# TDLdefA-QUN/Noise-Resilience-in-Discrete-Time-Crystal-Realizations-on-Quantum-Computers

Hardware: AMD Instinct MI355X
Metric: Floquet-periods×instances/sec at L=20; RZZ-kernel HBM GB/s vs peak (higher is better)
Workload: dtype f64

## Files before the change

noise-resilience-in-discrete-time-crystal-realizations-on-quantum-computers_amd/csrc/dtc_wavefront.hip:

```cpp
#include <hip/hip_runtime.h>

#include "dtc_device.h"
#include "dtc_kernels.h"
#include "dtc_wf_frame.h"

#ifndef DTC_WF_SPLIT
#define DTC_WF_SPLIT 1
#endif
#ifndef DTC_WF_WAVE_XCH
#define DTC_WF_WAVE_XCH 0
#endif
#ifndef DTC_WF_WG4
#define DTC_WF_WG4 1
#endif

namespace dtc {

template <int LAY>
__device__ __forceinline__ void wf_diag(double2 (&v)[kRegs], const double2* slot, int t,
                                        double2 fac, double2 e) {
  static_assert(LAY >= 0 && LAY <= 2, "tile layout");
  const double2 c = cmul(fac, e);
  const double2* tr = slot + (LAY == 1   ? wf_l1_reg_index(ybase<1>(t))
                              : LAY == 2 ? ((t >> 6) & 3)
                                         : ((t & 7) << 4));
  constexpr int kStep = LAY == 1 ? 2 : (LAY == 2 ? 4 : 1);
#pragma unroll
  for (int g = 0; g < kRegs; g += 4) {
#pragma unroll
    for (int r = g; r < g + 4; ++r) v[r] = cmul(v[r], cmul(c, tr[r * kStep]));
    __builtin_amdgcn_sched_barrier(0);
  }
}

template <int KIND>
__device__ __forceinline__ void wf_kick_lane3(double2 (&v)[kRegs], double f) {
  const long long sm = (KIND == kKindRY && (__lane_id() & 8)) ? (long long)(1ull << 63) : 0ll;
#pragma unroll
  for (int r = 0; r < kRegs; ++r) {
    const double px = xor_lane<8>(v[r].x), py = xor_lane<8>(v[r].y);
    if (KIND == kKindRX) {
      v[r] = make_double2(fma(f, v[r].x, -py), fma(f, v[r].y, px));
    } else {
      v[r] = make_double2(fma(f, v[r].x, __longlong_as_double(__double_as_longlong(px) ^ sm)),
                          fma(f, v[r].y, __longlong_as_double(__double_as_longlong(py) ^ sm)));
    }
  }
}

__host__ __device__ constexpr int wf_slot_ofs(bool two_lay, int st) {
  return two_lay ? st * kWfTabB : (st >> 1) * kWfTab + (st & 1) * kWfTabB;
}
__host__ __device__ constexpr int wf_tab_lds(bool two_lay) { return wf_slot_ofs(two_lay, kWfSteps + 1); }
static_assert(kWfTabB == 64 && kWfL1Reg == 64 && kWfTabA == kWfFetchTabA && (kWfSteps & 1) == 0,
              "the register tables of dtc_wf_frame.h");

__host__ __device__ constexpr bool wf_wg4(int qm0) {
  return ((DTC_WF_WG4 >> (qm0 == 8)) & 1) &&
         sizeof(double) * kHalfSlots + sizeof(double2) * wf_tab_lds(kWfT2Lay1 && qm0 == 8) <=
             160 * 1024 / 4;
}

template <int KIND, int QM0, bool SPLIT>
__global__ __launch_bounds__(kThreads, SPLIT ? (wf_wg4(QM0) ? 4 : 3) : 2) void dtc_wf_pass(WfArgs A) {
  constexpr bool kWg4 = SPLIT && wf_wg4(QM0);
  constexpr bool kTwoLay = kWfT2Lay1 && QM0 == 8;
  __shared__ double2 s_tile[SPLIT ? 1 : kTile];
  __shared__ double s_half[SPLIT ? kHalfSlots : 1];
  __shared__ double2 s_tab[kWg4 || !SPLIT ? wf_tab_lds(kTwoLay) : (kWfSteps + 1) * kWfTab];
  static_assert(!kWg4 || sizeof(s_half) + sizeof(s_tab) <= 160 * 1024 / 4, "four workgroups per CU");
  static_assert(wf_tab_lds(kTwoLay) <= (kWfSteps + 1) * kWfTab, "the padded form holds the tables");

  const int t = threadIdx.x;
  const int og = A.octet_bits;
  const int64_t b = og ? (((int64_t)blockIdx.y << 3) | (blockIdx.x & 7)) : (int64_t)blockIdx.y;
  const int64_t tile = og ? (int64_t)(blockIdx.x >> 3) : (int64_t)blockIdx.x;
  if (b >= A.batch) return;
  const int inst = (int)((A.batch_start + b) / A.n_traj);
  const int n = A.n_steps;
  constexpr int kOddLay = kTwoLay ? 1 : 0;

  TileMap M;
  M.c = A.c;
  M.s = A.s;
  M.cmask = (1 << A.c) - 1;
  const int mid = A.s - A.c;
  M.tbase = ((tile & (((int64_t)1 << mid) - 1)) << A.c) | ((tile >> mid) << (A.s + kTileBits - A.c));

  const int var = A.out_bit >= 0 ? (int)((M.tbase >> A.out_bit) & 1) : 0;
  const double2* tg = A.tab + ((int64_t)inst * (kWfSteps + 1) * 2 + var) * kWfTab;
  double2 stage[kWfSteps + 1];
#pragma unroll
  for (int st = 0; st <= kWfSteps; ++st) {
    const int lay = (st & 1) ? kOddLay : 2;
    stage[st] = make_double2(1.0, 0.0);
    if (t < wf_reg_size(lay) && ((A.dmask >> st) & 1))
      stage[st] = tg[st * 2 * kWfTab + wf_reg_base(lay) + t];
  }

  const int64_t sbase = state_base(b, A.state_len, og);
  const int64_t vofs = octet_spread(M.at(ybase<2>(t)), og);
  double2 v[kRegs];
  {
    const double2* src = A.src + sbase + vofs;
#pragma unroll
    for (int r = 0; r < kRegs; ++r) {
      const d2v w =
          __builtin_nontemporal_load((const d2v*)(src + octet_spread(M.rel(r << 8), og)));
      v[r] = make_double2(w.x, w.y);
    }
  }
  const RecScalar R0(A.recs + b * kRecPerState);
  const RecScalar R1(A.recs + ((int64_t)A.batch + b) * kRecPerState);
  const long long fxd = R1.bits(8 * kRecTotal + kWfMaskXD);
  const int fzx = R1.i(kRecTotal, kWfMaskZX);
  const int last = 31 - __builtin_clz(A.dmask | 1);
  auto wf_fetch = [&](auto lay, int st) {
    constexpr int LAY = decltype(lay)::value;
    double2 e = make_double2(1.0, 0.0);
    if ((A.dmask >> st) & 1) {
      const int fx = (int)(fxd >> (kTileBits * st)) & (kTile - 1);
      e = tg[st * 2 * kWfTab + wf_thr_fetch(LAY, ybase<LAY>(t), fx)];
      if (st == last && wf_thr_neg(LAY, ybase<LAY>(t), fzx & (kTile - 1)))
        e = make_double2(-e.x, -e.y);
    }
    return e;
  };
  using L0 = std::integral_constant<int, 0>;
  using L1 = std::integral_constant<int, 1>;
  using L2 = std::integral_constant<int, 2>;
  using LOdd = std::integral_constant<int, kOddLay>;
  double2 cn = wf_fetch(L2{}, 0);
  if (t < kWfTabA) {
    const int fz = fzx & (kTile - 1);
#pragma unroll
    for (int st = 0; st <= kWfSteps; ++st) {
      const int lay = (st & 1) ? kOddLay : 2;
      if (t >= wf_reg_size(lay) || !((A.dmask >> st) & 1)) continue;
      const int fx = (int)(fxd >> (kTileBits * st)) & (kTile - 1);
      const int j = t ^ wf_reg_xmask(lay, fx);
      const bool neg = st == last && (__popc(j & wf_reg_zmask(lay, fz)) & 1);
      s_tab[wf_slot_ofs(kTwoLay, st) + j] =
          neg ? make_double2(-stage[st].x, -stage[st].y) : stage[st];
    }
  }
  __syncthreads();

  double2 gf = cmul(make_double2(R0.d(kRecTotal, 0), R0.d(kRecTotal, 1)),
                    make_double2(R1.d(kRecTotal, 0), R1.d(kRecTotal, 1)));
  auto diag = [&](auto lay, int st, auto nlay, int nx) {
    if ((A.dmask >> st) & 1) {
      wf_diag<decltype(lay)::value>(v, s_tab + wf_slot_ofs(kTwoLay, st), t, gf, cn);
      gf = make_double2(1.0, 0.0);
    }
    if (nx <= kWfSteps) cn = wf_fetch(nlay, nx);
  };
  auto kick = [&](auto nib, int st) {
    constexpr int N = decltype(nib)::value;
    if (!(A.mask[st] & (0xFu << (4 * N)))) return;
    const RecScalar R(A.recs + ((int64_t)(st >> 1) * A.batch + b) * kRecPerState);
    apply_nibble<N, KIND, N == 0 ? QM0 : 15, true>(v, R, (st & 1) * kTileBits);
  };
  constexpr bool kWaveXch = DTC_WF_WAVE_XCH != 0;

  auto kick3 = [&](int st) {
    if (!(A.mask[st] & 8u)) return;
    const RecScalar R(A.recs + ((int64_t)(st >> 1) * A.batch + b) * kRecPerState);
    wf_kick_lane3<KIND>(v, R.d((st & 1) * kTileBits + 3, 3));
  };

  int st = 0;
#pragma unroll 1
  do {
    diag(L2{}, st, LOdd{}, st + 1);
    if (st < n) {
      kick(L2{}, st);
      xch_tile<SPLIT, 2, 1>(v, s_tile, s_half, t);
      kick(L1{}, st);
      if constexpr (kTwoLay) {
        kick3(st);
      } else {
        xch_tile<SPLIT, 1, 0, kWaveXch>(v, s_tile, s_half, t);
        kick(L0{}, st);
      }
      diag(LOdd{}, st + 1, L2{}, st + 2);
      if (st + 1 < n) {
        if constexpr (kTwoLay) {
          kick3(st + 1);
          kick(L1{}, st + 1);
        } else {
          kick(L0{}, st + 1);
          xch_tile<SPLIT, 0, 1, kWaveXch>(v, s_tile, s_half, t);
          kick(L1{}, st + 1);
        }
        xch_tile<SPLIT, 1, 2>(v, s_tile, s_half, t);
        kick(L2{}, st + 1);
      }
    }
    st += 2;
  } while (st <= n);
  if (n & 1) xch_tile<SPLIT, kOddLay, 2>(v, s_tile, s_half, t);
  if (!A.dmask) {
    const int fz = fzx & (kTile - 1);
    const double sg = (__popc(t & fz) & 1) ? -1.0 : 1.0;
#pragma unroll
    for (int r = 0; r < kRegs; ++r) {
      const double s = (__popc(r & (fz >> 8)) & 1) ? -sg : sg;
      v[r] = cmul(v[r], make_double2(s * gf.x, s * gf.y));
    }
  }
  {
    const int fx = (fzx >> 16) & (kTile - 1);
    const int xr = fx >> 8;
    double2* dst = A.dst + sbase + octet_spread(M.at(ybase<2>(t) ^ (fx & 255)), og);
#pragma unroll
    for (int r = 0; r < kRegs; ++r) {
      d2v x;
      x.x = v[r].x;
      x.y = v[r].y;
      __builtin_nontemporal_store(x, (d2v*)(dst + octet_spread(M.rel((r ^ xr) << 8), og)));
    }
  }
}

hipError_t launch_wavefront(const WfArgs& a, int kind, hipStream_t stream) {
  if (a.L_eff < kTileBits || a.L_eff > 32 || a.n_steps < 1 || a.n_steps > kWfSteps ||
      a.c < 0 || a.c > kTileBits || a.s < a.c || a.s + kTileBits - a.c > a.L_eff ||
      a.out_bit >= a.L_eff || a.batch < 1 || !a.tab || !a.recs || !a.src || !a.dst)
    return hipErrorInvalidValue;
  if (a.octet_bits && (a.octet_bits < 4 || a.octet_bits > a.L_eff)) return hipErrorInvalidValue;
  const bool cols3 = a.c == 3;
  if (!cols3 && a.c != kTileBits) return hipErrorInvalidValue;
  for (int st = 0; st < a.n_steps; ++st)
    if (a.mask[st] >> kTileBits || (cols3 && (a.mask[st] & 7u))) return hipErrorInvalidValue;
  if (a.dmask < 0 || a.dmask >> (a.n_steps + 1)) return hipErrorInvalidValue;
  const int n_tiles = 1 << (a.L_eff - kTileBits);
  const dim3 grid = a.octet_bits ? dim3(n_tiles * 8, (a.batch + 7) / 8) : dim3(n_tiles, a.batch);
  const dim3 block(kThreads);
  constexpr bool kSplit = DTC_WF_SPLIT != 0;
  if (kind == kKindRX) {
    if (cols3) hipLaunchKernelGGL((dtc_wf_pass<kKindRX, 8, kSplit>), grid, block, 0, stream, a);
    else hipLaunchKernelGGL((dtc_wf_pass<kKindRX, 15, kSplit>), grid, block, 0, stream, a);
  } else if (kind == kKindRY) {
    if (cols3) hipLaunchKernelGGL((dtc_wf_pass<kKindRY, 8, kSplit>), grid, block, 0, stream, a);
    else hipLaunchKernelGGL((dtc_wf_pass<kKindRY, 15, kSplit>), grid, block, 0, stream, a);
  } else {
    return hipErrorInvalidValue;
  }
  return hipGetLastError();
}

}
```

noise-resilience-in-discrete-time-crystal-realizations-on-quantum-computers_amd/csrc/dtc_wf_frame.h:

```cpp
#pragma once
#include <stdint.h>

#ifdef __HIPCC__
#define DTC_WF_HD __host__ __device__
#else
#define DTC_WF_HD
#endif

namespace dtc {

static constexpr int kWfFrameSteps = 4;
static constexpr int kWfFrameBits = 12;

struct WfFrame {
  double coef[kWfFrameSteps][kWfFrameBits];
  uint64_t xdiag;
  int zlast;
  int xend;
  int ph;
};

DTC_WF_HD inline int wf_step_bits(uint32_t mask, int act) {
  int m = 0;
  for (int n = 0; n < 3; ++n)
    if (mask & (0xFu << (4 * n))) m |= 0xF << (4 * n);
  return m & act;
}

DTC_WF_HD inline void wf_frame_walk(bool rx, int n_steps, const uint32_t* mask, int dmask,
                                    int act, const int (*var)[kWfFrameBits],
                                    const double (*coef)[kWfFrameBits], WfFrame& o) {
  auto form_a = [&](int st, int k) { return (var[st][k] >> 1) ^ 1; };
  auto zbit = [&](int st, int k) {
    return rx ? (var[st][k] & 1) : ((var[st][k] & 1) ^ form_a(st, k));
  };
  int last = n_steps;
  for (int st = 0; st < n_steps; ++st)
    if ((dmask >> st) & 1) last = st;
  if ((dmask >> n_steps) & 1) last = n_steps;
  int npost = 0;
  for (int st = last; st < n_steps; ++st) {
    const int bits = wf_step_bits(mask[st], act);
    for (int k = 0; k < kWfFrameBits; ++k)
      if ((bits >> k) & 1) npost ^= zbit(st, k) << k;
  }
  int x = 0, z = 0, ph = 0;
  o.xdiag = 0;
  o.zlast = 0;
  for (int st = 0; st <= n_steps; ++st) {
    if ((dmask >> st) & 1) o.xdiag |= (uint64_t)x << (kWfFrameBits * st);
    if (st == last) {
      o.zlast = z ^ npost;
      z = npost;
    }
    for (int k = 0; k < kWfFrameBits; ++k) {
      if (st < kWfFrameSteps) o.coef[st][k] = 0.0;
      if (st == n_steps || !((wf_step_bits(mask[st], act) >> k) & 1)) continue;
      const int fa = form_a(st, k), n2 = zbit(st, k);
      const double g = fa ? -coef[st][k] : coef[st][k];
      const int flip = ((rx ? z : (x ^ z)) >> k) & 1;
      o.coef[st][k] = flip ? -g : g;
      ph += (rx ? 3 * fa : 2 * fa) + 2 * flip;
      x ^= fa << k;
      ph += 2 * (n2 & (x >> k) & 1);
      z ^= n2 << k;
    }
  }
  for (int st = n_steps + 1; st < kWfFrameSteps; ++st)
    for (int k = 0; k < kWfFrameBits; ++k) o.coef[st][k] = 0.0;
  o.xend = x;
  o.ph = ph & 3;
}

static constexpr int kWfL1Reg = 64;
static constexpr int kWfL1Thr = 32;

DTC_WF_HD inline bool wf_l1_reg_bit(int k) { return k >= 4 && k <= 7; }
DTC_WF_HD inline int wf_l1_reg_pos(int k) { return (k >= 3 && k <= 8) ? k - 3 : -1; }
DTC_WF_HD inline int wf_l1_thr_pos(int k) { return k == 3 ? 0 : ((k >= 8 && k <= 11) ? k - 7 : -1); }
DTC_WF_HD inline int wf_l1_reg_index(int y) { return (y >> 3) & 63; }
DTC_WF_HD inline int wf_l1_thr_index(int y) { return ((y >> 3) & 1) | (((y >> 8) & 15) << 1); }
DTC_WF_HD inline int wf_l1_reg_zmask(int z) { return (z >> 3) & 63; }
DTC_WF_HD inline int wf_l1_thr_zmask(int z) { return ((z >> 9) & 7) << 2; }
DTC_WF_HD inline bool wf_l1_in_reg(int k, int k2) {
  return wf_l1_reg_bit(k) || (k2 >= 0 && wf_l1_reg_bit(k2));
}

static constexpr int kWfFetchTabA = 128;
DTC_WF_HD inline int wf_thr_staged(int lay, int y) {
  return lay == 2 ? (y & (kWfFetchTabA - 1)) : (lay == 0 ? ((y >> 6) & 63) : wf_l1_thr_index(y));
}
DTC_WF_HD inline int wf_thr_fetch(int lay, int y, int fx) {
  const int i = wf_thr_staged(lay, y);
  if (lay == 2) return i ^ (fx & (kWfFetchTabA - 1));
  if (lay == 0) return kWfFetchTabA + (i ^ ((fx >> 6) & 63));
  return kWfL1Reg + (i ^ wf_l1_thr_index(fx));
}
DTC_WF_HD inline bool wf_thr_neg(int lay, int y, int fz) {
  const int zm = lay == 2 ? (fz & 63) : (lay == 0 ? ((fz >> 6) & 63) : wf_l1_thr_zmask(fz));
  int p = wf_thr_staged(lay, y) & zm;
  p ^= p >> 4;
  p ^= p >> 2;
  p ^= p >> 1;
  return p & 1;
}
DTC_WF_HD inline int wf_reg_base(int lay) { return lay == 2 ? kWfFetchTabA : 0; }
DTC_WF_HD inline int wf_reg_size(int lay) { return lay == 0 ? kWfFetchTabA : 64; }
DTC_WF_HD inline int wf_reg_xmask(int lay, int fx) {
  return lay == 2 ? ((fx >> 6) & 63) : (lay == 0 ? (fx & (kWfFetchTabA - 1)) : wf_l1_reg_index(fx));
}
DTC_WF_HD inline int wf_reg_zmask(int lay, int fz) {
  return lay == 2 ? ((fz >> 6) & 63) : (lay == 0 ? (fz & 63) : wf_l1_reg_zmask(fz));
}

}
#undef DTC_WF_HD
```

Measured before the change: 301,500.

## Add opt-in swap-based tile layout for split QM0=15 pass and pad layout-0 tables

Adds an optional layout path for the split kernel when QM0 is 15. It uses in-register lane swaps plus a single half-precision-slot LDS exchange, with pairwise kicks, in place of two tile exchanges per step. This aims to cut LDS traffic and barriers. Separately, the layout-0 diagonal tables in LDS are now padded (one slot per 16) to reduce bank conflicts, which changes the table stride and LDS footprint. The new exchange path is behind a compile flag that defaults off, and a host-visible symbol reports which form was built.

New measurement: 306,300, median of 6. +1.6%, better.

```diff
diff --git a/noise-resilience-in-discrete-time-crystal-realizations-on-quantum-computers_amd/csrc/dtc_wavefront.hip b/noise-resilience-in-discrete-time-crystal-realizations-on-quantum-computers_amd/csrc/dtc_wavefront.hip
--- a/noise-resilience-in-discrete-time-crystal-realizations-on-quantum-computers_amd/csrc/dtc_wavefront.hip
+++ b/noise-resilience-in-discrete-time-crystal-realizations-on-quantum-computers_amd/csrc/dtc_wavefront.hip
@@ -13,17 +13,21 @@
 #ifndef DTC_WF_WG4
 #define DTC_WF_WG4 1
 #endif
+#ifndef DTC_WF_T1_SWAP
+#define DTC_WF_T1_SWAP 0
+#endif
 
 namespace dtc {
 
-template <int LAY>
+template <int LAY, bool T1Q = false>
 __device__ __forceinline__ void wf_diag(double2 (&v)[kRegs], const double2* slot, int t,
                                         double2 fac, double2 e) {
-  static_assert(LAY >= 0 && LAY <= 2, "tile layout");
+  static_assert(LAY >= 0 && LAY <= 2 && (!T1Q || LAY == 0), "tile layout");
   const double2 c = cmul(fac, e);
   const double2* tr = slot + (LAY == 1   ? wf_l1_reg_index(ybase<1>(t))
                               : LAY == 2 ? ((t >> 6) & 3)
-                                         : ((t & 7) << 4));
+                              : T1Q      ? wf_pad0(wf_t1_ybase(kWfLayQ, t) & 0x70)
+                                         : wf_pad0((t & 7) << 4));
   constexpr int kStep = LAY == 1 ? 2 : (LAY == 2 ? 4 : 1);
 #pragma unroll
   for (int g = 0; g < kRegs; g += 4) {
@@ -48,8 +52,30 @@
   }
 }
 
+template <int FROM, int TO>
+__device__ __forceinline__ void exchange_t1(double2 (&v)[kRegs], double* s_half, int t) {
+  int bf = wf_t1_slot(wf_t1_ybase(FROM, t)), bt = wf_t1_slot(wf_t1_ybase(TO, t));
+  asm volatile("" : "+v"(bf), "+v"(bt));
+#pragma unroll
+  for (int r = 0; r < kRegs; ++r) s_half[bf ^ wf_t1_slot(wf_t1_roff(FROM, r))] = v[r].x;
+  __syncthreads();
+#pragma unroll
+  for (int r = 0; r < kRegs; ++r) v[r].x = s_half[bt ^ wf_t1_slot(wf_t1_roff(TO, r))];
+  __syncthreads();
+#pragma unroll
+  for (int r = 0; r < kRegs; ++r) s_half[bf ^ wf_t1_slot(wf_t1_roff(FROM, r))] = v[r].y;
+  __syncthreads();
+#pragma unroll
+  for (int r = 0; r < kRegs; ++r) v[r].y = s_half[bt ^ wf_t1_slot(wf_t1_roff(TO, r))];
+}
+
+__device__ __forceinline__ void wf_t1_swap(double2 (&v)[kRegs]) {
+  swap_reg_lane<0, 16>(v);
+  swap_reg_lane<1, 32>(v);
+}
+
 __host__ __device__ constexpr int wf_slot_ofs(bool two_lay, int st) {
-  return two_lay ? st * kWfTabB : (st >> 1) * kWfTab + (st & 1) * kWfTabB;
+  return two_lay ? st * kWfTabB : (st >> 1) * (kWfTabB + kWfTabA0) + (st & 1) * kWfTabB;
 }
 __host__ __device__ constexpr int wf_tab_lds(bool two_lay) { return wf_slot_ofs(two_lay, kWfSteps + 1); }
 static_assert(kWfTabB == 64 && kWfL1Reg == 64 && kWfTabA == kWfFetchTabA && (kWfSteps & 1) == 0,
@@ -65,6 +91,7 @@
 __global__ __launch_bounds__(kThreads, SPLIT ? (wf_wg4(QM0) ? 4 : 3) : 2) void dtc_wf_pass(WfArgs A) {
   constexpr bool kWg4 = SPLIT && wf_wg4(QM0);
   constexpr bool kTwoLay = kWfT2Lay1 && QM0 == 8;
+  constexpr bool kT1Swap = DTC_WF_T1_SWAP != 0 && SPLIT && QM0 == 15;
   __shared__ double2 s_tile[SPLIT ? 1 : kTile];
   __shared__ double s_half[SPLIT ? kHalfSlots : 1];
   __shared__ double2 s_tab[kWg4 || !SPLIT ? wf_tab_lds(kTwoLay) : (kWfSteps + 1) * kWfTab];
@@ -117,12 +144,12 @@
   const int last = 31 - __builtin_clz(A.dmask | 1);
   auto wf_fetch = [&](auto lay, int st) {
     constexpr int LAY = decltype(lay)::value;
+    const int yb = (kT1Swap && LAY == 0) ? wf_t1_ybase(kWfLayQ, t) : ybase<LAY>(t);
     double2 e = make_double2(1.0, 0.0);
     if ((A.dmask >> st) & 1) {
       const int fx = (int)(fxd >> (kTileBits * st)) & (kTile - 1);
-      e = tg[st * 2 * kWfTab + wf_thr_fetch(LAY, ybase<LAY>(t), fx)];
-      if (st == last && wf_thr_neg(LAY, ybase<LAY>(t), fzx & (kTile - 1)))
-        e = make_double2(-e.x, -e.y);
+      e = tg[st * 2 * kWfTab + wf_thr_fetch(LAY, yb, fx)];
+      if (st == last && wf_thr_neg(LAY, yb, fzx & (kTile - 1))) e = make_double2(-e.x, -e.y);
     }
     return e;
   };
@@ -140,7 +167,7 @@
       const int fx = (int)(fxd >> (kTileBits * st)) & (kTile - 1);
       const int j = t ^ wf_reg_xmask(lay, fx);
       const bool neg = st == last && (__popc(j & wf_reg_zmask(lay, fz)) & 1);
-      s_tab[wf_slot_ofs(kTwoLay, st) + j] =
+      s_tab[wf_slot_ofs(kTwoLay, st) + (lay == 0 ? wf_pad0(j) : j)] =
           neg ? make_double2(-stage[st].x, -stage[st].y) : stage[st];
     }
   }
@@ -150,7 +177,8 @@
                     make_double2(R1.d(kRecTotal, 0), R1.d(kRecTotal, 1)));
   auto diag = [&](auto lay, int st, auto nlay, int nx) {
     if ((A.dmask >> st) & 1) {
-      wf_diag<decltype(lay)::value>(v, s_tab + wf_slot_ofs(kTwoLay, st), t, gf, cn);
+      constexpr int LAY = decltype(lay)::value;
+      wf_diag<LAY, kT1Swap && LAY == 0>(v, s_tab + wf_slot_ofs(kTwoLay, st), t, gf, cn);
       gf = make_double2(1.0, 0.0);
     }
     if (nx <= kWfSteps) cn = wf_fetch(nlay, nx);
@@ -161,6 +189,14 @@
     const RecScalar R(A.recs + ((int64_t)(st >> 1) * A.batch + b) * kRecPerState);
     apply_nibble<N, KIND, N == 0 ? QM0 : 15, true>(v, R, (st & 1) * kTileBits);
   };
+  auto kick_pair = [&](auto half, int st) {
+    constexpr int H = decltype(half)::value;
+    if (!(A.mask[st] & 0xF0u)) return;
+    const RecScalar R(A.recs + ((int64_t)(st >> 1) * A.batch + b) * kRecPerState);
+    const int k = (st & 1) * kTileBits + 4 + 2 * H;
+    layer_f<KIND, 2, 0>(v, R.d(k, 3));
+    layer_f<KIND, 2, 1>(v, R.d(k + 1, 3));
+  };
   constexpr bool kWaveXch = DTC_WF_WAVE_XCH != 0;
 
   auto kick3 = [&](int st) {
@@ -170,36 +206,69 @@
   };
 
   int st = 0;
+  if constexpr (kT1Swap) {
+    using H0 = std::integral_constant<int, 0>;
+    using H1 = std::integral_constant<int, 1>;
 #pragma unroll 1
-  do {
-    diag(L2{}, st, LOdd{}, st + 1);
-    if (st < n) {
-      kick(L2{}, st);
-      xch_tile<SPLIT, 2, 1>(v, s_tile, s_half, t);
-      kick(L1{}, st);
-      if constexpr (kTwoLay) {
-        kick3(st);
-      } else {
-        xch_tile<SPLIT, 1, 0, kWaveXch>(v, s_tile, s_half, t);
+    do {
+      diag(L2{}, st, L0{}, st + 1);
+      if (st < n) {
+        kick(L2{}, st);
+        wf_t1_swap(v);
+        kick_pair(H0{}, st);
+        exchange_t1<kWfLayL2s, kWfLayQs>(v, s_half, t);
+        kick_pair(H1{}, st);
+        wf_t1_swap(v);
         kick(L0{}, st);
+        diag(L0{}, st + 1, L2{}, st + 2);
+        if (st + 1 < n) {
+          kick(L0{}, st + 1);
+          wf_t1_swap(v);
+          kick_pair(H1{}, st + 1);
+          exchange_t1<kWfLayQs, kWfLayL2s>(v, s_half, t);
+          kick_pair(H0{}, st + 1);
+          wf_t1_swap(v);
+          kick(L2{}, st + 1);
+        }
       }
-      diag(LOdd{}, st + 1, L2{}, st + 2);
-      if (st + 1 < n) {
+      st += 2;
+    } while (st <= n);
+    if (n & 1) {
+      __syncthreads();
+      exchange_t1<kWfLayQ, kWfLayL2>(v, s_half, t);
+    }
+  } else {
+#pragma unroll 1
+    do {
+      diag(L2{}, st, LOdd{}, st + 1);
+      if (st < n) {
+        kick(L2{}, st);
+        xch_tile<SPLIT, 2, 1>(v, s_tile, s_half, t);
+        kick(L1{}, st);
         if constexpr (kTwoLay) {
-          kick3(st + 1);
-          kick(L1{}, st + 1);
+          kick3(st);
         } else {
-          kick(L0{}, st + 1);
-          xch_tile<SPLIT, 0, 1, kWaveXch>(v, s_tile, s_half, t);
-          kick(L1{}, st + 1);
+          xch_tile<SPLIT, 1, 0, kWaveXch>(v, s_tile, s_half, t);
+          kick(L0{}, st);
         }
-        xch_tile<SPLIT, 1, 2>(v, s_tile, s_half, t);
-        kick(L2{}, st + 1);
+        diag(LOdd{}, st + 1, L2{}, st + 2);
+        if (st + 1 < n) {
+          if constexpr (kTwoLay) {
+            kick3(st + 1);
+            kick(L1{}, st + 1);
+          } else {
+            kick(L0{}, st + 1);
+            xch_tile<SPLIT, 0, 1, kWaveXch>(v, s_tile, s_half, t);
+            kick(L1{}, st + 1);
+          }
+          xch_tile<SPLIT, 1, 2>(v, s_tile, s_half, t);
+          kick(L2{}, st + 1);
+        }
       }
-    }
-    st += 2;
-  } while (st <= n);
-  if (n & 1) xch_tile<SPLIT, kOddLay, 2>(v, s_tile, s_half, t);
+      st += 2;
+    } while (st <= n);
+    if (n & 1) xch_tile<SPLIT, kOddLay, 2>(v, s_tile, s_half, t);
+  }
   if (!A.dmask) {
     const int fz = fzx & (kTile - 1);
     const double sg = (__popc(t & fz) & 1) ? -1.0 : 1.0;
@@ -251,3 +320,6 @@
 }
 
 }
+
+extern "C" __attribute__((visibility("default"))) const int dtc_wf_t1_swap_form =
+    (DTC_WF_T1_SWAP != 0 && DTC_WF_SPLIT != 0) ? 1 : 0;
diff --git a/noise-resilience-in-discrete-time-crystal-realizations-on-quantum-computers_amd/csrc/dtc_wf_frame.h b/noise-resilience-in-discrete-time-crystal-realizations-on-quantum-computers_amd/csrc/dtc_wf_frame.h
--- a/noise-resilience-in-discrete-time-crystal-realizations-on-quantum-computers_amd/csrc/dtc_wf_frame.h
+++ b/noise-resilience-in-discrete-time-crystal-realizations-on-quantum-computers_amd/csrc/dtc_wf_frame.h
@@ -113,5 +113,27 @@
   return lay == 2 ? ((fz >> 6) & 63) : (lay == 0 ? (fz & 63) : wf_l1_reg_zmask(fz));
 }
 
+DTC_WF_HD constexpr int wf_pad0(int j) { return j + (j >> 4); }
+static constexpr int kWfTabA0 = (wf_pad0(kWfFetchTabA - 1) + 1 + 3) & ~3;
+
+enum { kWfLayL2 = 0, kWfLayL2s = 1, kWfLayQ = 2, kWfLayQs = 3 };
+
+DTC_WF_HD constexpr int wf_t1_ybase(int lay, int t) {
+  const int l03 = t & 15, l45 = (t >> 4) & 3, w = t >> 6;
+  if (lay == kWfLayL2) return t;
+  if (lay == kWfLayL2s) return l03 | (l45 << 8) | (w << 6);
+  const int q = ((l03 & 3) << 4) | ((l03 >> 2) << 8) | (w << 10);
+  return lay == kWfLayQ ? (q | (l45 << 6)) : (q | l45);
+}
+DTC_WF_HD constexpr int wf_t1_roff(int lay, int r) {
+  if (lay == kWfLayL2) return r << 8;
+  if (lay == kWfLayL2s) return ((r & 3) << 4) | ((r >> 2) << 10);
+  if (lay == kWfLayQ) return r;
+  return ((r & 3) << 6) | ((r >> 2) << 2);
+}
+DTC_WF_HD constexpr int wf_t1_slot(int y) {
+  return y ^ ((y >> 4) & 3) ^ (((y >> 8) & 3) << 2) ^ (((y >> 8) & 1) << 4);
+}
+
 }
 #undef DTC_WF_HD
```
